# rgl-epfl/differentiable-sdf-rendering

Measured on AMD Instinct MI355X. Metric: diff-renders/sec (fwd+bwd) 256^3 SDF, 512^2, 12 views, higher is better.
Workload: dtype f32; 1 GPU; no-tex-12-hq sizes: 256^3 SDF, 12 views x 512^2, sdf_silhouette_reparam, spp primal/grad 256/64 (reference semantics, configs.py:16,19); views_total=12, views_this_rank=12, partition=whole views, spp_primal=256, spp_grad=64, schedule=primal pass and gradient sweep on two HIP streams

## Files before the change

### differentiable-sdf-rendering_amd/csrc/dsdf_items_body.h

```cpp
    static_assert(!STORE_T || !DIRECT, "STORE_T is a mode of the one-channel marches");
    constexpr int NCH = DIRECT ? 4 : 2;
    __shared__ __attribute__((aligned(16))) float wave_lds[DSDF_WAVE_LDS];
    const int lid = lane_id();
    const uint32_t npix = (uint32_t)(VB.v[0].Wb * VB.v[0].Hb);
    const uint32_t chunks = (uint32_t)__builtin_amdgcn_readfirstlane(VB.v[0].spp >> 6);
    const uint32_t n_items = (uint32_t)__builtin_amdgcn_readfirstlane((int)items[0]) * chunks;
    WaveStats wst = {0, 0, 0, 0, 0, 0, 0};
    const uint32_t sub = (blockIdx.x >> 3) & 7u, first = gridDim.x / DSDF_TICKETS;
    uint32_t share = blockIdx.x & 7u, hops = 0;
    const uint32_t my_subq = tail_subq();
    auto draw = [&](uint32_t sh) { return ticket_draw(items, sh, sub, first); };
    uint32_t item = item_of(share, blockIdx.x >> 3), next = 0;
    if (lid == 0) next = draw(share);
    while (true) {
        if (item >= n_items) {
            if (++hops == 8u) break;
            share = (share + 1u) & 7u;
            if (lid == 0) next = draw(share);
            item = (uint32_t)__builtin_amdgcn_readfirstlane((int)next);
            if (lid == 0) next = draw(share);
            continue;
        }
      {
        const uint32_t e = (uint32_t)__builtin_amdgcn_readfirstlane((int)list[item / chunks]);
        const uint32_t view = e / npix, pix = e - view * npix;
        const ViewArgs &A = VB.v[view];
        float *__restrict__ block = blocks + (size_t)view * NCH * npix;
        const int py = (int)(pix / (uint32_t)A.Wb), px = (int)(pix - (uint32_t)py * (uint32_t)A.Wb);
        const unsigned proof = skip ? (unsigned)__builtin_amdgcn_readfirstlane((int)skip[e]) : 0u;
        const bool skip_trace = (proof & (DIFF ? DSDF_PX_EMPTY_G : DSDF_PX_EMPTY)) != 0;
        const bool known_hit = !DIFF && !DIRECT && (proof & DSDF_PX_HIT) && A.integrator == DSDF_SILHOUETTE;
        const uint32_t unit = pix * chunks + item % chunks;
        const uint32_t lane = unit * 64u + (uint32_t)lid;
        auto hand_off = [&tq, my_subq, item, view, lane](auto &ho) { ho.tq = tq; ho.sub = tq.per_xcd ? my_subq : item % DSDF_TAIL_SUBQ; ho.view = view; ho.lane = lane; };
        TraceOut tr, trs, trb;
        clear_trace(tr);
        int lit = 0;
        float acc[NCH][2], win[4] = {0.f, 0.f, 0.f, 0.f};
#pragma unroll
        for (int ch = 0; ch < NCH; ++ch) { acc[ch][0] = 0.f; acc[ch][1] = 0.f; }
        const bool proven = !DIFF && !DIRECT && !STORE_T && (known_hit || skip_trace);
        Lane L;
        if (STORE_T) {
            if (!skip_trace) {
                L = lane_setup<!DIFF>(A, P, lane, px, py);
                if (DIFF) {
                    DirectFetch F;
                    if (tq.state) {
                        HandOff ho;
                        hand_off(ho);
                        trace_diff(G, P, L.ray.o, L.ray.d, L.ray.maxt, tr, F, ho);
                    } else trace_diff(G, P, L.ray.o, L.ray.d, L.ray.maxt, tr, F);
                    const Queue qv = view_queue(qall, view);
                    store_record(qv.rec + lane, qv.cap, tr);
                } else {
                    WaveCellCache F; F.taps = wave_lds; F.lid = lid;
                    if (tq.state) {
                        PlainHandOff ho;
                        hand_off(ho);
                        trace_plain(G, P, L.ray.o, L.ray.d, L.ray.maxt, tr, F, ho);
                    } else trace_plain(G, P, L.ray.o, L.ray.d, L.ray.maxt, tr, F);
                    hit_t[hit_slot(npix, A.spp, view, lane)] = tr.its_t;
                }
            }
        } else if (proven) {
            float r0, r1;
            sample_offsets(A, lane, r0, r1);
            film_accum_offsets(r0, r1, known_hit ? 1.f : 0.f, wave_lds, lid, win);
            if (known_hit) tr.its_t = 0.f;
        } else {
        L = lane_setup<!DIFF>(A, P, lane, px, py);
        if (known_hit) tr.its_t = 0.f;
        else if (!skip_trace) {
            if (DIFF) {
                DirectFetch F;
                if (!DIRECT && tq.state) {
                    HandOff ho;
                    hand_off(ho);
                    trace_diff(G, P, L.ray.o, L.ray.d, L.ray.maxt, tr, F, ho);
                } else trace_diff(G, P, L.ray.o, L.ray.d, L.ray.maxt, tr, F);
            } else {
                WaveCellCache F; F.taps = wave_lds; F.lid = lid;
                if (!DIRECT && tq.state) {
                    PlainHandOff ho;
                    hand_off(ho);
                    trace_plain(G, P, L.ray.o, L.ray.d, L.ray.maxt, tr, F, ho);
                } else trace_plain(G, P, L.ray.o, L.ray.d, L.ray.maxt, tr, F);
            }
        }
        if (DIRECT) {
            const Reproj rp = reproject(A.cam, P, L.ray.o + L.ray.d, A.W, A.H);
            float rgb[3];
            lit = direct_value(G, P, A, S, L, lane, tr.its_t, DIFF, trs, trb, rgb);
            film_accum_wave<NCH>(px, py, rp.u, rp.v, rgb, wave_lds, lid, acc);
        } else if (DIFF) {
            const Reproj rp = reproject(A.cam, P, L.ray.o + L.ray.d, A.W, A.H);
            const float val = shade_value(G, A, L, tr.its_t);
            film_accum_wave<NCH>(px, py, rp.u, rp.v, &val, wave_lds, lid, acc);
        } else {
            const float val = shade_value(G, A, L, tr.its_t);
            film_accum_offsets(L.r0, L.r1, val, wave_lds, lid, win);
        }
        }
        if (DIRECT || DIFF) { if (!STORE_T) film_flush_wave<NCH>(block, A, px, py, lid, acc); }
        else if (!STORE_T) film_flush_mfma(block, A, px, py, lid, win);
        bool need = false;
        if (DIFF && !STORE_T) {
            need = needs_backward<DIRECT>(G, P, A, L, tr, lit);
            queue_unit(view_queue(qall, view), unit, lane, need, lid, tr, DIRECT ? &trs : nullptr, (DIRECT && S.use_mis) ? &trb : nullptr);
        }
        if (STATS) add_stats(wst, tr, true, need);
        if (STATS && DIRECT) {
            wst.ssteps += wave_sum_i32(trs.steps); wst.swsteps += wave_max_i32(trs.steps); wst.srays += wave_sum_i32(trs.steps > 0 ? 1 : 0);
        }
      }
        item = (uint32_t)__builtin_amdgcn_readfirstlane((int)next);
        if (lid == 0) next = draw(share);
    }
    if (STATS) flush_stats(stats, wst, blockIdx.x, lid);
```

### differentiable-sdf-rendering_amd/csrc/dsdf_kernels.hip

```cpp
#include <hip/hip_runtime.h>
#include <stdio.h>
#include <stdlib.h>
#include <string.h>
#include <mutex>
#include <vector>
#include "dsdf_lane.h"

using namespace dsdf;

#if DSDF_XF
namespace dsdf {
__constant__ XfState g_xf_dev;
XfState g_xf_host = {{1.f, 0.f, 0.f, 0.f, 1.f, 0.f, 0.f, 0.f, 1.f}, {0.f, 0.f, 0.f}, {0.f, 0.f, 0.f}, {1.f, 1.f, 1.f}};
}
#endif

#define DSDF_BLOCK 256
#define DSDF_TSTRIDE 68
#define DSDF_TROWS 13
#define DSDF_WAVE_LDS 1104
#ifndef DSDF_PRIMAL_MINWAVES
#define DSDF_PRIMAL_MINWAVES 8
#endif

// ... 201 lines not shown
}

#define DSDF_ITEM_REGION 16384
#define DSDF_TICKETS 64
#define DSDF_ITEM_HDR (16 + 16 * DSDF_TICKETS)
__device__ __forceinline__ uint32_t ticket_draw(uint32_t *items, uint32_t sh, uint32_t sub, uint32_t first) {
    return item_of(sh, sub + 8u * (first + atomicAdd(items + 16 + 16 * (sh * 8u + sub), 1u)));
}
struct ItemOrder { int tw_log2, th_log2; uint32_t tiles_x, per_view; };

__global__ __launch_bounds__(256) void k_build_items(ViewBatch VB, int view0, int nv, const unsigned char *__restrict__ skip, unsigned far_bit,
                                                     int row0, int row1, ItemOrder O, uint32_t *__restrict__ hdr, uint32_t *__restrict__ list) {
    const ViewArgs &A = VB.v[0];
    const uint32_t npix = (uint32_t)(A.Wb * A.Hb), total = O.per_view * (uint32_t)nv;
    const uint32_t begin = blockIdx.x * DSDF_ITEM_REGION;
    const int w = threadIdx.x >> 6, lid = lane_id();
    __shared__ uint32_t wcount[4];
    __shared__ uint32_t base;
    auto entry = [&](uint32_t i) -> uint32_t {
        if (i >= total) return ~0u;
        const uint32_t gv = i / O.per_view, r = i - gv * O.per_view, view = (uint32_t)view0 + gv;
        const uint32_t tile = r >> (O.tw_log2 + O.th_log2), in = r & ((1u << (O.tw_log2 + O.th_log2)) - 1u);
        const uint32_t ty = tile / O.tiles_x, tx = tile - ty * O.tiles_x;
        const int px = (int)((tx << O.tw_log2) + (in & ((1u << O.tw_log2) - 1u))), py = (int)((ty << O.th_log2) + (in >> O.tw_log2));
        if (px >= A.Wb || py >= A.Hb || py < row0 || py >= row1) return ~0u;
        const uint32_t e = view * npix + (uint32_t)py * (uint32_t)A.Wb + (uint32_t)px;
        return (skip && (skip[e] & far_bit)) ? ~0u : e;
    };
    auto live = [&](uint32_t i) { return entry(i) != ~0u; };
    uint32_t mine = 0;
    for (uint32_t o = 0; o < DSDF_ITEM_REGION; o += 256) mine += live(begin + o + threadIdx.x) ? 1u : 0u;
    const uint32_t wsum = (uint32_t)wave_sum_i32((int)mine);
    if (lid == 0) wcount[w] = wsum;
    __syncthreads();
    if (threadIdx.x == 0) {
        const uint32_t t = wcount[0] + wcount[1] + wcount[2] + wcount[3];
        base = t ? atomicAdd(hdr, t) : 0u;
    }
    __syncthreads();
    uint32_t run = base;
    for (uint32_t o = 0; o < DSDF_ITEM_REGION; o += 256) {
        const uint32_t e = entry(begin + o + threadIdx.x);
        const bool l = e != ~0u;
        const uint64_t m = __ballot(l);
        __syncthreads();
        if (lid == 0) wcount[w] = (uint32_t)__popcll(m);
        __syncthreads();
        uint32_t before = 0, all = 0;
#pragma unroll
        for (int k = 0; k < 4; ++k) { const uint32_t c = wcount[k]; before += k < w ? c : 0u; all += c; }
        if (l) list[run + before + mask_prefix(m)] = e;
        run += all;
    }
}

#ifndef DSDF_DIRECT_PRIMAL_MINWAVES
#define DSDF_DIRECT_PRIMAL_MINWAVES 1
#endif
#ifndef DSDF_DIRECT_SWEEP_MINWAVES
#define DSDF_DIRECT_SWEEP_MINWAVES 1
#endif
template <bool DIFF, bool DIRECT, bool STATS>
__global__ __launch_bounds__(64, DIRECT ? (DIFF ? DSDF_DIRECT_SWEEP_MINWAVES : DSDF_DIRECT_PRIMAL_MINWAVES) : (DIFF ? DSDF_DIFF_MINWAVES : DSDF_PRIMAL_MINWAVES))
void k_render_items(GridView G, dsdf_params P, ViewBatch VB, float *__restrict__ blocks, Queue qall, unsigned long long *stats,
                    const unsigned char *__restrict__ skip, ShadeArgs S, TailQueue tq, uint32_t *__restrict__ items,
                    const uint32_t *__restrict__ list) {
    constexpr bool STORE_T = false;
    float *const hit_t = nullptr;
#include "dsdf_items_body.h"
}
template <bool DIFF, bool STATS>
__global__ __launch_bounds__(64, DIFF ? DSDF_DIFF_MINWAVES : DSDF_PRIMAL_MINWAVES)
void k_render_items_store(GridView G, dsdf_params P, ViewBatch VB, Queue qall, unsigned long long *stats, const unsigned char *__restrict__ skip,
                          ShadeArgs S, TailQueue tq, uint32_t *__restrict__ items, const uint32_t *__restrict__ list, float *__restrict__ hit_t) {
    constexpr bool DIRECT = false, STORE_T = true;
    float *const blocks = nullptr;
#include "dsdf_items_body.h"
}

template <int PHASE, bool DIFF>
__global__ __launch_bounds__(64) void k_direct_items(GridView G, dsdf_params P, ViewBatch VB, float *__restrict__ blocks,
                                                     const unsigned char *__restrict__ skip, ShadeArgs S, TailQueue sq, uint32_t *__restrict__ items,
                                                     const uint32_t *__restrict__ list, float *__restrict__ hit_t, Queue qall) {
    constexpr int NCH = 4;
    __shared__ __attribute__((aligned(16))) float wave_lds[DSDF_WAVE_LDS];
    const int lid = lane_id();
    const uint32_t npix = (uint32_t)(VB.v[0].Wb * VB.v[0].Hb);
    const uint32_t chunks = (uint32_t)__builtin_amdgcn_readfirstlane(VB.v[0].spp >> 6);
    const uint32_t per_item = (PHASE == 1 && !DIFF) ? chunks : 1u;
    const uint32_t n_items = (uint32_t)__builtin_amdgcn_readfirstlane((int)items[0]) * (chunks / per_item);
    const uint32_t sub = (blockIdx.x >> 3) & 7u, first = gridDim.x / DSDF_TICKETS;
    uint32_t share = blockIdx.x & 7u, hops = 0;
    const uint32_t my_subq = tail_subq();
    auto draw = [&](uint32_t sh) { return ticket_draw(items, sh, sub, first); };
    uint32_t item = item_of(share, blockIdx.x >> 3), next = 0;
    if (lid == 0) next = draw(share);
    while (true) {
        if (item >= n_items) {
            if (++hops == 8u) break;
            share = (share + 1u) & 7u;
            if (lid == 0) next = draw(share);
            item = (uint32_t)__builtin_amdgcn_readfirstlane((int)next);
            if (lid == 0) next = draw(share);
            continue;
        }
        {
// ... 937 lines not shown
    const ViewBatch &VB;
    int nv;
    GridView G;
    ShadeArgs S;
    Queue q;
    float *film;
    const unsigned char *skip;
    unsigned long long *st64;
    bool deep_skip;
    bool env_fill;
};

template <bool DIFF>
static int prefill_film(const PassCtx &c, const Batch &b) {
    int rc;
    const dim3 grid((unsigned)((c.Wb * c.Hb + 255) / 256), b.nv), blk(256);
    if (b.deep_skip && (rc = launch("k_film_ones", k_film_ones, grid, blk, c.st, b.VB, b.skip, b.film, c.row0, c.row1, b.st64))) return rc;
    if (b.env_fill && (rc = launch("k_film_env", k_film_env, grid, blk, c.st, b.VB, b.skip, b.film, c.row0, c.row1,
                                   DIFF ? DSDF_PX_EMPTY_G : DSDF_PX_EMPTY, b.S.env[0], b.S.env[1], b.S.env[2])))
        return rc;
    return DSDF_OK;
}

template <bool DIFF>
static int persistent_pass(PassCtx &c, const Workspace &ws, const Batch &b, bool wavefront) {
    int rc;
    hipStream_t st = c.st;
    const int nv = b.nv;
    const unsigned far_bit = (c.direct && !b.S.hide_emitters && !b.env_fill) ? 0u : (DIFF ? DSDF_PX_FAR_G : (DSDF_PX_FAR | (b.deep_skip ? DSDF_PX_DEEP : 0u)));
    if (hipMemsetAsync(ws.items, 0, (size_t)DSDF_MAX_GROUPS * DSDF_ITEM_HDR * sizeof(uint32_t), st) != hipSuccess)
        return fail(DSDF_ERR_LAUNCH, "hipMemsetAsync(work list) failed");
    ItemOrder O;
    {
        unsigned tile_px = DSDF_ITEM_SEG / (unsigned)(c.spp / 64);
        if (tile_px < 1) tile_px = 1;
        int lg = 0;
        while ((2u << lg) <= tile_px) ++lg;
        O.tw_log2 = (lg + 1) / 2; O.th_log2 = lg / 2;
        O.tiles_x = (unsigned)((c.Wb + (1u << O.tw_log2) - 1) >> O.tw_log2);
        const unsigned tiles_y = (unsigned)((c.Hb + (1u << O.th_log2) - 1) >> O.th_log2);
        O.per_view = (O.tiles_x * tiles_y) << (O.tw_log2 + O.th_log2);
    }
    if (DIFF && hipMemsetAsync(ws.count, 0, (size_t)nv * ws.nunits * sizeof(uint32_t), st) != hipSuccess)
        return fail(DSDF_ERR_LAUNCH, "hipMemsetAsync(queue counts) failed");
    const bool handoff = ws.tail != nullptr && (!c.direct || wavefront);
    const size_t cnt_bytes = align_up((size_t)DSDF_MAX_GROUPS * DSDF_TAIL_SUBQ * DSDF_TAIL_CNT_STRIDE * sizeof(uint32_t), 256);
    if (handoff && hipMemsetAsync(ws.tail, 0, cnt_bytes, st) != hipSuccess)
        return fail(DSDF_ERR_LAUNCH, "hipMemsetAsync(tail queue) failed");
    uint32_t *hdr = ws.items;
    uint32_t *list = ws.items + (size_t)DSDF_MAX_GROUPS * DSDF_ITEM_HDR;
    if ((rc = launch("k_build_items", k_build_items, dim3((unsigned)(((size_t)nv * O.per_view + DSDF_ITEM_REGION - 1) / DSDF_ITEM_REGION)), dim3(256), st,
                     b.VB, 0, nv, b.skip, far_bit, c.row0, c.row1, O, hdr, list)))
        return rc;
    TailQueue tq;
    memset(&tq, 0, sizeof(tq));
    if (handoff) {
        tq.cap_sub = ws.tail_cap_sub * (uint32_t)((nv + ws.group_views - 1) / ws.group_views);
        tq.per_xcd = 1u;
        tq.count = (uint32_t *)ws.tail;
        tq.state = (float *)(ws.tail + cnt_bytes);
    }
    const GridView &G = b.G;
    const ShadeArgs &S = b.S;
    const Queue &q = b.q;
    unsigned long long *st64 = b.st64;
    const dim3 grid(worker_blocks()), blk(64);
    timing_mark(0, st);
    if (wavefront)
        rc = launch("k_render_items", st64 ? k_render_items_store<DIFF, true> : k_render_items_store<DIFF, false>, grid, blk, st,
                    G, c.pp, b.VB, q, st64, b.skip, S, tq, hdr, list, ws.hit_t);
    else
        rc = launch("k_render_items", c.direct ? (st64 ? k_render_items<DIFF, true, true> : k_render_items<DIFF, true, false>)
                                               : (st64 ? k_render_items<DIFF, false, true> : k_render_items<DIFF, false, false>),
                    grid, blk, st, G, c.pp, b.VB, b.film, q, st64, b.skip, S, tq, hdr, list);
    if (rc) return rc;
    timing_mark(1, st);
    if (!handoff) return DSDF_OK;
    bool coef_beside = false;
    hipEvent_t coef_fork = nullptr;
    hipStream_t hs[2] = {st, st};
    if (DIFF && c.coef_beside && ws.count0 && helper_streams(st, hs)) {
        if (hipMemcpyAsync(ws.count0, ws.count, (size_t)nv * ws.nunits * sizeof(uint32_t), hipMemcpyDeviceToDevice, st) != hipSuccess)
            return fail(DSDF_ERR_LAUNCH, "hipMemcpyAsync(queue lengths) failed");
        coef_beside = true;
        coef_fork = next_event();
        if (!coef_fork || hipEventRecord(coef_fork, st) != hipSuccess) return fail(DSDF_ERR_LAUNCH, "coefficient stream fork failed");
    }
    const dim3 tgrid(DSDF_TAIL_SUBQ * DSDF_TAIL_BLOCKS_PER_SUBQ), tblk(256);
    unsigned long long *tst = wavefront ? nullptr : (st64 ? st64 : g_tail_stats);
    if (DIFF) rc = launch("k_tail_trace", wavefront ? k_tail_trace_diff<true> : k_tail_trace_diff<false>, tgrid, tblk, st, G, c.pp, b.VB, b.film, tq, q, tst);
    else rc = launch("k_tail_trace", k_tail_trace_plain, tgrid, tblk, st, G, c.pp, b.VB, b.film, tq, tst, wavefront ? ws.hit_t : nullptr);
    if (rc) return rc;
    if (coef_beside) {
        hipStream_t cs = hs[1];
        if (hipStreamWaitEvent(cs, coef_fork, 0) != hipSuccess) return fail(DSDF_ERR_LAUNCH, "coefficient stream fork failed");
        const dim3 cgrid((ws.nunits + DSDF_BWD_UNITS - 1) / DSDF_BWD_UNITS, nv);
        if ((rc = launch("k_backward_coef", k_backward_coef, cgrid, dim3(64), cs, G, c.pp, b.VB, q, nullptr, nullptr, ws.count0))) return rc;
        hipEvent_t join = next_event();
        if (!join || hipEventRecord(join, cs) != hipSuccess) return fail(DSDF_ERR_LAUNCH, "coefficient stream join failed");
        c.coef_done_early = true;
        if (hipStreamWaitEvent(st, join, 0) != hipSuccess) return fail(DSDF_ERR_LAUNCH, "tail stream join failed");
    }
    return DSDF_OK;
}

template <bool DIFF>
// ... 359 lines not shown
```

### differentiable-sdf-rendering_amd/csrc/dsdf_math.h

```cpp
#pragma once
#include <math.h>
#include <stdint.h>
#include "../../include/dsdf.h"

#if defined(__HIPCC__)
#define DSDF_HD __host__ __device__ __forceinline__
#else
#define DSDF_HD inline
#endif

#ifndef DSDF_FAST_RCP
#define DSDF_FAST_RCP 1
#endif

namespace dsdf {

struct V3 { float x, y, z; };
DSDF_HD V3 mk(float x, float y, float z) { V3 r; r.x = x; r.y = y; r.z = z; return r; }
DSDF_HD V3 operator+(V3 a, V3 b) { return mk(a.x + b.x, a.y + b.y, a.z + b.z); }
DSDF_HD V3 operator-(V3 a, V3 b) { return mk(a.x - b.x, a.y - b.y, a.z - b.z); }
DSDF_HD V3 operator-(V3 a) { return mk(-a.x, -a.y, -a.z); }
DSDF_HD V3 operator*(V3 a, float s) { return mk(a.x * s, a.y * s, a.z * s); }
DSDF_HD V3 operator*(float s, V3 a) { return mk(a.x * s, a.y * s, a.z * s); }
DSDF_HD V3 operator*(V3 a, V3 b) { return mk(a.x * b.x, a.y * b.y, a.z * b.z); }
// ... 579 lines not shown
            float w = eval_trace_weight(P, d, i, lo, hi, x, v, g, H, w_d);
            float inv_den = rcpf_s<1>(fminf(P.extra_thresh, sd));
            float diff = prev_sd - sd;
            ews += (diff >= 0.f) ? diff * inv_den : 0.f;
            ews = fminf(ews, 1.f);
            float cur = hit ? 0.f : sd;
            float seg = 0.5f * (cur + prev_sd);
            float winc = seg * w * ews;
            wsum += winc;
            warp_t += winc * t;
            w_d = fma3(dot(d, w_d), t_d, t * w_d);
            V3 gc = fma3(dot(d, g), t_d, t * g);
            V3 seg_d = 0.5f * (gc + prev_gc);
            V3 sd_d = drsign(v) * gc;
            V3 ewd = (prev_gc - sd_d) * inv_den;
            if (v < P.extra_thresh) ewd = ewd - (diff * inv_den * inv_den) * sd_d;
            if (diff > 0.f) ews_d = ews_d + ewd;
            if (ews >= 1.f || ews <= 0.f) ews_d = mk(0.f, 0.f, 0.f);
            w_d = w * ews_d + ews * w_d;
            w *= ews;
            V3 winc_d = w * seg_d + seg * w_d;
            mixed = mixed + t * winc_d + (w * seg) * t_d;
            t_d = t_d + gc;
            wdsum = wdsum + winc_d;
            ++i;
            t += cur;
            prev_sd = sd;
            prev_gc = gc;
            active = (t <= maxt) && !hit;
        }
    }
    C.leftover(active, t, warp_t, prev_sd, wsum, ews, t_d, prev_gc, mixed, wdsum, ews_d, i);
    out.steps = i;
    out.weight_sum = wsum;
    out.its_t = refine_hit(G, P, o, d, its_t, trace_eps, out.refine_steps, F);
    float inv = 1.f / wsum;
    warp_t *= inv;
    V3 warp_t_d = (mixed - warp_t * wdsum) * inv;
    float ww = fminf(fmaxf(wsum, 0.f), 1.f);
    V3 ww_d = (wsum > 0.f && wsum < 1.f) ? wdsum : mk(0.f, 0.f, 0.f);
    bool invalid = (wsum < 1e-7f) || !hit_box || active;
    if (invalid) {
        warp_t = INFINITY; warp_t_d = mk(0.f, 0.f, 0.f); ww = 0.f; ww_d = mk(0.f, 0.f, 0.f);
    }
    out.warp_t = warp_t; out.warp_t_d = warp_t_d; out.warp_weight = ww; out.warp_weight_d = ww_d;
}

template <class Fetch>
DSDF_HD void trace_diff(const GridView &G, const dsdf_params &P, V3 o, V3 d_in, float ray_maxt, TraceOut &out, Fetch &F) {
    MarchToEnd C;
    trace_diff(G, P, o, d_in, ray_maxt, out, F, C);
}

struct DiffMarch {
    V3 o, d;
    float t, maxt, trace_eps, its_t;
    float warp_t, prev_sd, wsum, ews;
    V3 t_d, prev_gc, mixed, wdsum, ews_d;
    int i;
    bool active, hit_box;
};

DSDF_HD DiffMarch diff_march_begin(const dsdf_params &P, V3 o, V3 d_in, float ray_maxt) {
    DiffMarch m;
    float invn = rsqf_s<2>(dot(d_in, d_in));
    m.o = o;
    m.d = d_in * invn;
    const BoxBound lo = box_lo(P), hi = box_hi(P);
    BoxHit b = bbox_ray_intersect(lo, hi, o, m.d);
    m.hit_box = b.hit && (b.mint > 0.f || b.inside);
    m.active = m.hit_box;
    m.maxt = fminf(b.maxt, ray_maxt);
    m.trace_eps = P.trace_eps * fmaxf(m.maxt, 1.f);
    m.its_t = INFINITY;
    m.t = b.inside ? 0.f : b.mint + 1e-5f;
    m.warp_t = 0.f; m.prev_sd = 0.f; m.wsum = 0.f; m.ews = 0.f;
    m.prev_gc = mk(0.f, 0.f, 0.f); m.mixed = mk(0.f, 0.f, 0.f); m.wdsum = mk(0.f, 0.f, 0.f); m.ews_d = mk(0.f, 0.f, 0.f);
    m.i = 0;
    V3 pb = fma3(m.t, m.d, o);
    V3 n = closest_axis(box_face_distance(lo, hi, pb));
    float ddn = dot(m.d, n);
    m.t_d = mk(0.f, 0.f, 0.f);
    if (!b.inside && fabsf(ddn) > 0.f) m.t_d = n * (-m.t / ddn);
    return m;
}

DSDF_HD void diff_march_step(const dsdf_params &P, DiffMarch &m, V3 x, float v, V3 g, const float H[6]) {
    const BoxBound lo = box_lo(P), hi = box_hi(P);
    const V3 d = m.d;
    const float t = m.t;
    bool hit = v < m.trace_eps;
    if (hit) m.its_t = t;
    float sd = fabsf(v);
    V3 w_d;
    float w = eval_trace_weight(P, d, m.i, lo, hi, x, v, g, H, w_d);
    float inv_den = rcpf_s<1>(fminf(P.extra_thresh, sd));
    float diff = m.prev_sd - sd;
    m.ews += (diff >= 0.f) ? diff * inv_den : 0.f;
    m.ews = fminf(m.ews, 1.f);
    float cur = hit ? 0.f : sd;
    float seg = 0.5f * (cur + m.prev_sd);
    float winc = seg * w * m.ews;
    m.wsum += winc;
    m.warp_t += winc * t;
    w_d = fma3(dot(d, w_d), m.t_d, t * w_d);
    V3 gc = fma3(dot(d, g), m.t_d, t * g);
// ... 425 lines not shown
```

### differentiable-sdf-rendering_amd/python/dsdf/_lib.py

```python
import ctypes as C
import os

_HERE = os.path.dirname(os.path.abspath(__file__))
LIB_PATH = os.environ.get('DSDF_LIB_PATH') or os.path.normpath(os.path.join(_HERE, '..', '..', 'lib', 'libdsdf.so'))

DSDF_SILHOUETTE = 0
DSDF_SIMPLE_SHADING = 1
DSDF_DIRECT = 2
DSDF_REPARAM = 1
DSDF_NO_SKIP = 2
DSDF_NO_HIT_PROOF = 4


class DsdfCamera(C.Structure):
    _fields_ = [('origin', C.c_float * 3), ('left', C.c_float * 3), ('up', C.c_float * 3),
                ('dir', C.c_float * 3), ('tan_half_fov', C.c_float), ('pad', C.c_float * 3)]


class DsdfParams(C.Structure):
    _fields_ = [('trace_eps', C.c_float), ('extra_thresh', C.c_float), ('sil_weight_offset', C.c_float),
                ('sil_weight_epsilon', C.c_float), ('bbox_delta', C.c_float), ('edge_eps', C.c_float),
                ('clamping_thresh', C.c_float), ('near_clip', C.c_float), ('far_clip', C.c_float),
                ('sdf_p', C.c_float * 3), ('weight_strategy', C.c_int), ('refine_steps', C.c_int),
                ('light_dir', C.c_float * 3), ('normalize_warp_field', C.c_int), ('max_reparam_depth', C.c_int)]


class DsdfShading(C.Structure):
    _fields_ = [('albedo', C.c_void_p), ('ax', C.c_int), ('ay', C.c_int), ('az', C.c_int),
                ('env_radiance', C.c_float * 3), ('hide_emitters', C.c_int), ('emitter_samples', C.c_void_p),
                ('grad_albedo', C.c_void_p), ('use_mis', C.c_int), ('variant', C.c_int), ('bsdf_samples', C.c_void_p),
                ('bsdf', C.c_int), ('roughness', C.c_void_p), ('rax', C.c_int), ('ray', C.c_int), ('raz', C.c_int),
                ('grad_roughness', C.c_void_p), ('bsdf_lobe_samples', C.c_void_p)]


class DsdfError(RuntimeError):
    pass


_lib = None
ABI_VERSION = 308

SYMBOLS = {
    'dsdf_version': (C.c_int, []),
    'dsdf_share_pixel_skip': (C.c_int, [C.c_void_p, C.c_size_t]),
    'dsdf_kernel_timing_arm': (C.c_int, []),
    'dsdf_tail_stats_arm': (C.c_int, [C.c_void_p]),
    'dsdf_kernel_timing_read': (C.c_int, [C.POINTER(C.c_float)]),
    'dsdf_last_error': (C.c_char_p, []),
    'dsdf_default_params': (None, [C.POINTER(DsdfParams)]),
    'dsdf_padded_size': (C.c_size_t, [C.c_int, C.c_int, C.c_int]),
    'dsdf_pad_grid': (C.c_int, [C.c_void_p, C.c_int, C.c_int, C.c_int, C.c_void_p, C.c_void_p]),
    'dsdf_eval_cubic': (C.c_int, [C.c_void_p, C.c_int, C.c_int, C.c_int, C.POINTER(DsdfParams), C.c_void_p,
                                  C.c_int64, C.c_int, C.c_void_p, C.c_void_p, C.c_void_p, C.c_void_p]),
    'dsdf_trace': (C.c_int, [C.c_void_p, C.c_int, C.c_int, C.c_int, C.POINTER(DsdfParams), C.c_void_p, C.c_void_p,
                             C.c_void_p, C.c_int64, C.c_int, C.c_void_p, C.c_void_p, C.c_void_p, C.c_void_p,
                             C.c_void_p, C.c_void_p, C.c_void_p]),
    'dsdf_warp_eval': (C.c_int, [C.c_void_p, C.c_int, C.c_int, C.c_int, C.POINTER(DsdfParams), C.c_void_p, C.c_void_p, C.c_int64,
                                 C.c_void_p, C.c_void_p, C.c_void_p, C.c_void_p, C.c_void_p, C.c_void_p, C.c_void_p, C.c_void_p,
                                 C.c_void_p, C.c_void_p]),
    'dsdf_surface_interaction': (C.c_int, [C.c_void_p, C.c_int, C.c_int, C.c_int, C.POINTER(DsdfParams), C.c_void_p, C.c_void_p,
                                           C.c_void_p, C.c_int64, C.c_void_p, C.c_void_p, C.c_void_p, C.c_void_p, C.c_void_p]),
    'dsdf_render_workspace_size': (C.c_size_t, [C.c_int, C.c_int, C.c_int, C.c_int, C.c_int]),
    'dsdf_forward_workspace_size': (C.c_size_t, [C.c_int, C.c_int, C.c_int, C.c_int, C.c_int]),
    'dsdf_cell_table_size': (C.c_size_t, [C.c_int, C.c_int, C.c_int]),
# ... 92 lines not shown
```

### differentiable-sdf-rendering_amd/python/dsdf/renderer.py

```python
import contextlib
import ctypes as C

import os

import torch

from . import _lib
from ._lib import (DSDF_DIRECT, DSDF_NO_HIT_PROOF, DSDF_NO_SKIP, DSDF_REPARAM, DSDF_SILHOUETTE, DSDF_SIMPLE_SHADING, DsdfCamera,
                   DsdfShading)

INTEGRATORS = {'sdf_silhouette_reparam': DSDF_SILHOUETTE, 'sdf_simple_shading_reparam': DSDF_SIMPLE_SHADING,
               'sdf_direct_reparam': DSDF_DIRECT,
               DSDF_SILHOUETTE: DSDF_SILHOUETTE, DSDF_SIMPLE_SHADING: DSDF_SIMPLE_SHADING, DSDF_DIRECT: DSDF_DIRECT}

STAT_NAMES = ('lanes', 'bbox_lanes', 'steps', 'hits', 'refine_steps', 'warp_active', 'queue_len', 'wave_steps',
              'tail_steps', 'tail_wave_steps', 'tail_rays')
STAT_SLOTS = 16

_workspaces = {}


def _proof_flags(empty_space_skip):
    if empty_space_skip == 'empty-only':
        return DSDF_NO_HIT_PROOF
    return 0 if empty_space_skip else DSDF_NO_SKIP

MAX_VIEWS_PER_LAUNCH = 16


def _stream():
    return C.c_void_p(torch.cuda.current_stream().cuda_stream)


def _ptr(t):
    return C.c_void_p(t.data_ptr()) if t is not None else C.c_void_p(0)


def _floats(a):
    return (C.c_float * len(a))(*[float(v) for v in a])


def _as_list(sensors):
    return list(sensors) if isinstance(sensors, (list, tuple)) else [sensors]


def _require_dev(t, name, dtype=torch.float32):
    if not isinstance(t, torch.Tensor) or not t.is_cuda:
        raise _lib.DsdfError(f"{name} must be a torch tensor on the HIP device (got {type(t).__name__}"
                             f"{'' if not isinstance(t, torch.Tensor) else ' on ' + str(t.device)}); no CPU path exists")
    if t.dtype != dtype:
        raise _lib.DsdfError(f"{name} must be {dtype}, got {t.dtype}")
    return t.contiguous()


def _workspace(device, nbytes, min_bytes=None):
    ws = _workspaces.get(device)
    if ws is not None and ws.numel() >= nbytes:
        return ws
    _workspaces.pop(device, None)
    del ws
    want = int(nbytes)
    while True:
        try:
            ws = torch.empty(want, dtype=torch.uint8, device=device)
            break
        except torch.OutOfMemoryError:
            if min_bytes is None or want <= int(min_bytes):
                raise
            torch.cuda.empty_cache()
            want = max(int(min_bytes), want // 2)
    _workspaces[device] = ws
    return ws


def release_workspaces():
    _workspaces.clear()
    _sweep_workspaces.clear()

# ... 209 lines not shown
    lib = grid.lib()
    rays_o = _require_dev(rays_o, 'rays_o'); rays_d = _require_dev(rays_d, 'rays_d'); t = _require_dev(t, 't')
    n = rays_o.shape[0]
    dev = rays_o.device
    f = lambda *s: torch.empty(*s, dtype=torch.float32, device=dev)
    out = dict(p=f(n, 3), n=f(n, 3), grad=f(n, 3), t_coef=f(n))
    with torch.cuda.device(dev):
        _lib.check(lib.dsdf_surface_interaction(_ptr(grid.padded), grid.rx, grid.ry, grid.rz, C.byref(grid.params), _ptr(rays_o),
                                                _ptr(rays_d), _ptr(t), n, _ptr(out['p']), _ptr(out['n']), _ptr(out['grad']),
                                                _ptr(out['t_coef']), _stream()))
    return out


def _views(sensors):
    sensors = _as_list(sensors)
    W, H = sensors[0].film_size()
    for s in sensors:
        if s.film_size() != (W, H):
            raise _lib.DsdfError("all sensors of one call must share the film size")
    cams = (DsdfCamera * len(sensors))(*[s.to_struct() for s in sensors])
    return sensors, cams, W, H


def _sampler_args(n_views, seeds, offsets, n_lanes):
    cseeds = None
    if seeds is not None:
        seeds = [seeds] * n_views if isinstance(seeds, int) else list(seeds)
        if len(seeds) != n_views:
            raise _lib.DsdfError("one seed per view is required")
        cseeds = (C.c_uint32 * n_views)(*[int(s) & 0xffffffff for s in seeds])
    if offsets is not None:
        offsets = _require_dev(offsets, 'offsets')
        if offsets.numel() != n_views * n_lanes * 2:
            raise _lib.DsdfError(f"offsets must hold n_views*(W+4)*(H+4)*spp*2 = {n_views * n_lanes * 2} floats, "
                                 f"got {offsets.numel()}")
        return offsets, cseeds
    if cseeds is None:
        raise _lib.DsdfError("either seeds or offsets is required")
    return None, cseeds


class _Call:

    def __init__(self, grid, sensors, spp, seeds=None, offsets=None, integrator=DSDF_SILHOUETTE, reparam=True, empty_space_skip=True,
                 shading=None, emitter_samples=None, bsdf_samples=None, grad_albedo=None):
        self.grid, self.params = grid, grid.params
        self.extended = _needs_extended(shading)
        self.lib = grid.lib(self.extended)
        self.sensors, self.cams, self.W, self.H = _views(sensors)
        self.nv, self.spp = len(self.sensors), int(spp)
        self.n_lanes = (self.W + 4) * (self.H + 4) * self.spp
        self.offsets, self.cseeds = _sampler_args(self.nv, seeds, offsets, self.n_lanes)
        self.integrator = INTEGRATORS[integrator]
        self.flags = (DSDF_REPARAM if reparam else 0) | _proof_flags(empty_space_skip)
        self.sh = self._keep = None
        if self.integrator == DSDF_DIRECT:
            if shading is None:
                raise _lib.DsdfError("sdf_direct_reparam needs shading=dsdf.Shading(albedo, ...)")
            st, keep = shading.to_struct(self.nv, self.n_lanes, emitter_samples, grad_albedo, bsdf_samples)
            self.sh, self._keep = C.byref(st), (st, keep)

    def args(self):
        g = self.grid
        return (_ptr(g.padded), g.rx, g.ry, g.rz, C.byref(self.params), self.cams, self.nv, self.W, self.H, self.spp,
                _ptr(self.offsets), self.cseeds, self.integrator, self.flags, self.sh)

    def workspace(self, diff):
        size = self.lib.dsdf_render_workspace_size if diff else self.lib.dsdf_forward_workspace_size
        extra = 0
        if not diff and self.integrator == DSDF_DIRECT:
            extra = int(self.lib.dsdf_cell_table_size(self.grid.rx, self.grid.ry, self.grid.rz)) + 256
        return _workspace(self.grid.device, size(self.W, self.H, self.spp, min(self.nv, MAX_VIEWS_PER_LAUNCH), self.integrator) + extra,
                          size(self.W, self.H, self.spp, 1, self.integrator))

    def image(self, wanted=True):
        return torch.empty(self.nv, self.H, self.W, 3, dtype=torch.float32, device=self.grid.device) if wanted else None

    def run(self, entry, *tail):
        with torch.cuda.device(self.grid.device):
            _lib.check(getattr(self.lib, entry)(*self.args(), *tail, _stream()))


def sampler_offsets(sensors, spp, seeds, mirror=False, device=None):
    lib = _lib.load()
    sensors, _, W, H = _views(sensors)
    nv = len(sensors)
    n_lanes = (W + 4) * (H + 4) * int(spp)
    _, cseeds = _sampler_args(nv, seeds, None, n_lanes)
    dev = torch.device('cuda', torch.cuda.current_device()) if device is None else torch.device(device)
    out = torch.empty(nv, n_lanes, 2, dtype=torch.float32, device=dev)
    with torch.cuda.device(dev):
        _lib.check(lib.dsdf_sampler_2d(cseeds, nv, W, H, int(spp), int(bool(mirror)), _ptr(out), _stream()))
    return out


def render_forward(grid, sensors, spp, seeds=None, offsets=None, integrator=DSDF_SILHOUETTE, reparam=True, stats=None,
                   empty_space_skip=True, shading=None, emitter_samples=None, bsdf_samples=None):
    c = _Call(grid, sensors, spp, seeds, offsets, integrator, reparam, empty_space_skip, shading, emitter_samples, bsdf_samples)
    img = c.image()
    ws = c.workspace(False)
    c.run('dsdf_render_forward', _ptr(img), _ptr(ws), ws.numel(), _ptr(stats))
    return img


AOV_NAMES = ['sdf_value', 'warp_t', 'vx', 'vy', 'div', 'i', 'weight_sum', 'weight', 'warp_t_dx', 'warp_t_dy', 'warp_t_dz']


# ... 291 lines not shown
            _lib.check(lib.dsdf_redistance_status(_ptr(ws), rx, ry, rz, _ptr(status), _stream()))
            return out.reshape(shape), status
    return out.reshape(shape)


def mesh_raycast(triangles, rays_o, rays_d, t_min=0.0):
    lib = _lib.load()
    tri = _require_dev(triangles.reshape(-1, 9), 'triangles')
    rays_o = _require_dev(rays_o, 'rays_o'); rays_d = _require_dev(rays_d, 'rays_d')
    n = rays_o.shape[0]
    t = torch.empty(n, dtype=torch.float32, device=rays_o.device)
    back = torch.empty(n, dtype=torch.int32, device=rays_o.device)
    with torch.cuda.device(rays_o.device):
        _lib.check(lib.dsdf_mesh_raycast(_ptr(tri), int(tri.shape[0]), _ptr(rays_o), _ptr(rays_d), n, C.c_float(t_min), _ptr(t), _ptr(back),
                                         _stream()))
    return t, back


def kernel_timing_arm():
    _lib.check(_lib.load().dsdf_kernel_timing_arm())


def kernel_timing_read():
    ms = C.c_float(0.0)
    _lib.check(_lib.load().dsdf_kernel_timing_read(C.byref(ms)))
    return float(ms.value)


def tail_stats_arm(stats):
    global _tail_stats_held
    if stats is not None and (stats.dtype != torch.int64 or stats.numel() < 64 * STAT_SLOTS or not stats.is_contiguous()):
        raise ValueError("tail_stats_arm: a contiguous int64 tensor of 64 x STAT_SLOTS counters (new_stats()) is expected")
    for lib in {id(l): l for l in (_lib.load(), *_lib._variants.values())}.values():
        _lib.check(lib.dsdf_tail_stats_arm(_ptr(stats) if stats is not None else None))
    _tail_stats_held = stats


_tail_stats_held = None


def new_stats(device):
    return torch.zeros(64, STAT_SLOTS, dtype=torch.int64, device=device)


def stats_dict(stats):
    tot = [int(x) for x in stats.sum(0).cpu()]
    d = dict(zip(STAT_NAMES, tot))
    d['all_steps'] = d['steps'] + d['tail_steps']
    rows = [[int(x) for x in stats[r].cpu()] for r in range(4)]
    r0, r1 = rows[0], rows[1]
    d['tail_waves'] = {'max_wave_steps': r0[11], 'max_us': r0[12] / 100.0, 'sum_us': r0[13] / 100.0, 'sum_clocks': r0[14],
                       'sum_refill_clocks': r0[15], 'refills': r1[11], 'clocks_completing': r1[12], 'clocks_claiming': r1[13],
                       'clocks_setting_up': r1[14], 'idle_lanes_at_refill': r1[15]}
    M = (1 << 64) - 1
    for name, r in (('primal_tail', rows[2]), ('sweep_tail', rows[3])):
        if r[12]:
            t0 = M - (r[11] & M)
            d['tail_waves'][name] = {'latest_start_us': (r[12] - t0) / 100.0, 'earliest_end_us': ((M - (r[13] & M)) - t0) / 100.0,
                                     'latest_end_us': (r[14] - t0) / 100.0, 'first_start_tick': t0}
    return d


def eager_sweep_enabled():
    return os.environ.get('DSDF_EAGER_SWEEP', '1') != '0'


class _RenderOp(torch.autograd.Function):

    @staticmethod
    def forward(ctx, data, grid, sensors, spp, seed, spp_grad, seed_grad, integrator, reparam, p=None, albedo=None,
                shading=None, roughness=None):
        if albedo is not None:
            shading = shading.with_albedo(albedo)
        ctx.data_shape = data.shape
        ctx.p_meta = None if p is None else (p.shape, p.dtype, p.device)
        if not grid.in_sync_with(data):
            grid.update(data)
        if p is not None:
            grid.set_translation(p)
        n = len(sensors)
        sh = shading
        want_r = sh is not None and sh.roughness is not None and roughness is not None and ctx.needs_input_grad[12]
        want_a = sh is not None and (ctx.needs_input_grad[10] or want_r)
        ctx.ga = torch.zeros_like(sh.albedo.detach(), dtype=torch.float32).contiguous() if want_a else None
        ctx.gr = None
        if want_r:
            ctx.gr = sh.grad_roughness = torch.zeros_like(sh.roughness.detach(), dtype=torch.float32).contiguous()
        ctx.gp = torch.zeros(3, dtype=torch.float32, device=grid.device) if (p is not None and ctx.needs_input_grad[9]) else None
        ctx.grid = grid
        ctx.version = grid.version
        ctx.n_backward = 0
        if not eager_sweep_enabled():
            ctx.step = None
            ctx.lazy = (list(sensors), int(spp_grad), [seed_grad + i for i in range(n)], integrator, reparam, sh, grid.version)
            return render_forward(grid, sensors, spp, seeds=[seed + i for i in range(n)], integrator=integrator, reparam=reparam, shading=sh)
        img, ctx.step = step_begin(grid, sensors, spp, spp_grad, [seed + i for i in range(n)], [seed_grad + i for i in range(n)],
                                   integrator, reparam, sh, ctx.ga)
        return img

    @staticmethod
    def backward(ctx, grad_out):
        if ctx.version != ctx.grid.version:
            raise _lib.DsdfError("the grid was updated between this render and its backward: back-propagate before the optimiser step")
        if ctx.n_backward > 0:
            for t in (ctx.gp, ctx.ga, ctx.gr):
                if t is not None:
# ... 34 lines not shown
```

### include/dsdf.h

```cpp
#ifndef DSDF_H
#define DSDF_H

#include <stddef.h>
#include <stdint.h>

#ifdef __cplusplus
extern "C" {
#endif

#define DSDF_VERSION 308
#define DSDF_STAT_SLOTS 16

enum dsdf_status {
    DSDF_OK = 0,
    DSDF_ERR_INVALID_ARG = -1,
    DSDF_ERR_WORKSPACE = -2,
    DSDF_ERR_LAUNCH = -3,
    DSDF_ERR_NO_DEVICE = -4
};

enum dsdf_integrator {
    DSDF_SILHOUETTE = 0,
    DSDF_SIMPLE_SHADING = 1,
    DSDF_DIRECT = 2
};

enum dsdf_flags {
    DSDF_REPARAM = 1,
    DSDF_NO_SKIP = 2,
    DSDF_NO_HIT_PROOF = 4
};

typedef struct dsdf_camera {
    float origin[3];
    float left[3];
    float up[3];
    float dir[3];
    float tan_half_fov;
    float pad[3];
} dsdf_camera;

typedef struct dsdf_params {
    float trace_eps;
    float extra_thresh;
    float sil_weight_offset;
    float sil_weight_epsilon;
    float bbox_delta;
    float edge_eps;
    float clamping_thresh;
    float near_clip;
    float far_clip;
    float sdf_p[3];
    int   weight_strategy;
    int   refine_steps;
    float light_dir[3];
    int   normalize_warp_field;
    int   max_reparam_depth;
} dsdf_params;

typedef struct dsdf_shading {
    const float *albedo;
    int   ax, ay, az;
    float env_radiance[3];
    int   hide_emitters;
    const float *emitter_samples;
    float *grad_albedo;
    int   use_mis;
    int   variant;
    const float *bsdf_samples;
    int   bsdf;
    const float *roughness;
    int   rax, ray, raz;
    float *grad_roughness;
    const float *bsdf_lobe_samples;
} dsdf_shading;

int         dsdf_version(void);
const char *dsdf_last_error(void);
void        dsdf_default_params(dsdf_params *p);

size_t dsdf_padded_size(int rx, int ry, int rz);

int dsdf_pad_grid(const float *data, int rx, int ry, int rz, float *padded, void *stream);
// ... 101 lines not shown
```

Before: 29.41 renders/s.

## Probe gradient-sweep pixels with a capped lite march to skip full diff traces

Adds a probe kernel that, after item lists are built, traces one representative ray per pixel with a cheap capped sphere march (no derivative tracking) and marks items whose rays finish and need no backward work. In the gradient sweep, marked items first run the lite march per lane. If the whole wave finishes and needs no backward pass, the full differentiable trace and queueing are skipped; otherwise the wave falls back to the full trace. This aims to cut expensive trace_diff work on pixels far from silhouettes. The cost is an extra probe launch, redundant lite marches for chunks that fall back, and reliance on one probe ray being representative of all of a pixel's samples.

```diff
diff --git a/differentiable-sdf-rendering_amd/csrc/dsdf_items_body.h b/differentiable-sdf-rendering_amd/csrc/dsdf_items_body.h
--- a/differentiable-sdf-rendering_amd/csrc/dsdf_items_body.h
+++ b/differentiable-sdf-rendering_amd/csrc/dsdf_items_body.h
@@ -1,5 +1,7 @@
     static_assert(!STORE_T || !DIRECT, "STORE_T is a mode of the one-channel marches");
     constexpr int NCH = DIRECT ? 4 : 2;
+    constexpr bool LITE = DIFF && !DIRECT && !STORE_T;
+    int lite_wsteps = 0, lite_fallbacks = 0;
     __shared__ __attribute__((aligned(16))) float wave_lds[DSDF_WAVE_LDS];
     const int lid = lane_id();
     const uint32_t npix = (uint32_t)(VB.v[0].Wb * VB.v[0].Hb);
@@ -22,7 +24,8 @@
             continue;
         }
       {
-        const uint32_t e = (uint32_t)__builtin_amdgcn_readfirstlane((int)list[item / chunks]);
+        const uint32_t e_raw = (uint32_t)__builtin_amdgcn_readfirstlane((int)list[item / chunks]);
+        const uint32_t e = LITE ? e_raw & ~DSDF_ITEM_LITE : e_raw;
         const uint32_t view = e / npix, pix = e - view * npix;
         const ViewArgs &A = VB.v[view];
         float *__restrict__ block = blocks + (size_t)view * NCH * npix;
@@ -41,6 +44,7 @@
         for (int ch = 0; ch < NCH; ++ch) { acc[ch][0] = 0.f; acc[ch][1] = 0.f; }
         const bool proven = !DIFF && !DIRECT && !STORE_T && (known_hit || skip_trace);
         Lane L;
+        bool lite_done = false;
         if (STORE_T) {
             if (!skip_trace) {
                 L = lane_setup<!DIFF>(A, P, lane, px, py);
@@ -70,8 +74,23 @@
             if (known_hit) tr.its_t = 0.f;
         } else {
         L = lane_setup<!DIFF>(A, P, lane, px, py);
+        if (LITE && (e_raw & DSDF_ITEM_LITE) && !skip_trace) {
+#if DSDF_LITE_CACHE
+            WaveCellCache F; F.taps = wave_lds; F.lid = lid;
+#else
+            DirectFetch F;
+#endif
+            MarchCapped cap = {(A.flags & DSDF_REPARAM) ? DSDF_LITE_CAP : 0x7fffffff};
+            const bool fin = trace_lite(G, P, L.ray.o, L.ray.d, L.ray.maxt, tr, F, cap);
+            lite_done = __ballot(!fin || needs_backward<false>(G, P, A, L, tr, 0)) == 0;
+            if (STATS) {
+                const int it = wave_max_i32(tr.steps) + wave_max_i32(tr.refine_steps);
+                lite_wsteps += it;
+                if (!lite_done) { wst.steps += wave_sum_i32(tr.steps); wst.wsteps += it; ++lite_fallbacks; }
+            }
+        }
         if (known_hit) tr.its_t = 0.f;
-        else if (!skip_trace) {
+        else if (!skip_trace && !lite_done) {
             if (DIFF) {
                 DirectFetch F;
                 if (!DIRECT && tq.state) {
@@ -106,7 +125,7 @@
         else if (!STORE_T) film_flush_mfma(block, A, px, py, lid, win);
         bool need = false;
         if (DIFF && !STORE_T) {
-            need = needs_backward<DIRECT>(G, P, A, L, tr, lit);
+            need = !lite_done && needs_backward<DIRECT>(G, P, A, L, tr, lit);
             queue_unit(view_queue(qall, view), unit, lane, need, lid, tr, DIRECT ? &trs : nullptr, (DIRECT && S.use_mis) ? &trb : nullptr);
         }
         if (STATS) add_stats(wst, tr, true, need);
@@ -118,3 +137,7 @@
         if (lid == 0) next = draw(share);
     }
     if (STATS) flush_stats(stats, wst, blockIdx.x, lid);
+    if (STATS && LITE && lid == 0 && lite_wsteps) {
+        atomicAdd(stats + DSDF_STAT_LITE_ROW * DSDF_STAT_SLOTS + 11, (unsigned long long)lite_wsteps);
+        atomicAdd(stats + DSDF_STAT_LITE_ROW * DSDF_STAT_SLOTS + 12, (unsigned long long)lite_fallbacks);
+    }
diff --git a/differentiable-sdf-rendering_amd/csrc/dsdf_kernels.hip b/differentiable-sdf-rendering_amd/csrc/dsdf_kernels.hip
--- a/differentiable-sdf-rendering_amd/csrc/dsdf_kernels.hip
+++ b/differentiable-sdf-rendering_amd/csrc/dsdf_kernels.hip
@@ -277,6 +277,31 @@
         if (l) list[run + before + mask_prefix(m)] = e;
         run += all;
     }
+}
+
+#define DSDF_ITEM_LITE 0x80000000u
+#ifndef DSDF_LITE_CACHE
+#define DSDF_LITE_CACHE 1
+#endif
+__global__ __launch_bounds__(256) void k_warp_probe(GridView G, dsdf_params P, ViewBatch VB, const unsigned char *__restrict__ skip,
+                                                    const uint32_t *__restrict__ hdr, uint32_t *__restrict__ list, int mark_all) {
+    const uint32_t i = blockIdx.x * 256u + threadIdx.x;
+    if (i >= hdr[0]) return;
+    const uint32_t e = list[i];
+    bool mark = mark_all != 0;
+    if (!mark && !(skip && (skip[e] & DSDF_PX_EMPTY_G))) {
+        const uint32_t npix = (uint32_t)(VB.v[0].Wb * VB.v[0].Hb);
+        const uint32_t view = e / npix, pix = e - view * npix;
+        const ViewArgs &A = VB.v[view];
+        const int py = (int)(pix / (uint32_t)A.Wb), px = (int)(pix - (uint32_t)py * (uint32_t)A.Wb);
+        const Lane L = lane_setup(A, P, pix * (uint32_t)A.spp, px, py);
+        DirectFetch F;
+        MarchCapped cap = {DSDF_LITE_CAP};
+        TraceOut tr;
+        const bool fin = trace_lite(G, P, L.ray.o, L.ray.d, L.ray.maxt, tr, F, cap);
+        mark = fin && !needs_backward<false>(G, P, A, L, tr, 0);
+    }
+    if (mark) list[i] = e | DSDF_ITEM_LITE;
 }
 
 #ifndef DSDF_DIRECT_PRIMAL_MINWAVES
@@ -1320,6 +1345,11 @@
     if ((rc = launch("k_build_items", k_build_items, dim3((unsigned)(((size_t)nv * O.per_view + DSDF_ITEM_REGION - 1) / DSDF_ITEM_REGION)), dim3(256), st,
                      b.VB, 0, nv, b.skip, far_bit, c.row0, c.row1, O, hdr, list)))
         return rc;
+    const int lite = (DIFF && !c.direct && !wavefront && (size_t)nv * c.Wb * c.Hb < 0x80000000ull && !(c.flags & DSDF_SWEEP_LITE_OFF))
+                         ? ((c.flags & DSDF_SWEEP_LITE_ALL) ? 2 : 1) : 0;
+    if (lite > 0 && (rc = launch("k_warp_probe", k_warp_probe, dim3((unsigned)(((size_t)nv * c.Wb * c.Hb + 255) / 256)), dim3(256), st,
+                                 b.G, c.pp, b.VB, b.skip, hdr, list, (int)(lite >= 2))))
+        return rc;
     TailQueue tq;
     memset(&tq, 0, sizeof(tq));
     if (handoff) {
diff --git a/differentiable-sdf-rendering_amd/csrc/dsdf_math.h b/differentiable-sdf-rendering_amd/csrc/dsdf_math.h
--- a/differentiable-sdf-rendering_amd/csrc/dsdf_math.h
+++ b/differentiable-sdf-rendering_amd/csrc/dsdf_math.h
@@ -655,6 +655,85 @@
     trace_diff(G, P, o, d_in, ray_maxt, out, F, C);
 }
 
+template <class B>
+DSDF_HD float eval_trace_weight_lite(const dsdf_params &P, V3 d, int i, B lo, B hi, V3 x, float v, V3 g) {
+    float n_dot_d = dot(g, d);
+    float n_dot_n = dot(g, g);
+    float ratio = n_dot_d * rcpf_s<0>(n_dot_n);
+    float denom = P.sil_weight_epsilon + fabsf(v) + P.sil_weight_offset * n_dot_d * ratio;
+    float inv_denom = rcpf_s<0>(denom);
+    float dist_w = inv_denom * inv_denom * inv_denom;
+    V3 bd_d;
+    float bd = bbox_distance_inside_d(x, lo, hi, bd_d);
+    const float bbox_eps = 0.01f;
+    float bw = i > 0 ? fminf(bd, bbox_eps) * (1.f / bbox_eps) : 1.f;
+    return dist_w * bw;
+}
+
+struct MarchCapped {
+    int left;
+    template <class Fetch> DSDF_HD bool more(const Fetch &F, bool active) { return F.any(active) && left-- > 0; }
+};
+#ifndef DSDF_LITE_CAP
+#define DSDF_LITE_CAP 64
+#endif
+
+template <class Fetch, class Ctl>
+DSDF_HD bool trace_lite(const GridView &G, const dsdf_params &P, V3 o, V3 d_in, float ray_maxt, TraceOut &out, Fetch &F, Ctl &C) {
+    float invn = rsqf_s<2>(dot(d_in, d_in));
+    V3 d = d_in * invn;
+    const BoxBound lo = box_lo(P), hi = box_hi(P);
+    BoxHit b = bbox_ray_intersect(lo, hi, o, d);
+    bool hit_box = b.hit && (b.mint > 0.f || b.inside);
+    bool active = hit_box;
+    float maxt = fminf(b.maxt, ray_maxt);
+    float trace_eps = P.trace_eps * fmaxf(maxt, 1.f);
+    float its_t = INFINITY;
+    float t = b.inside ? 0.f : b.mint + 1e-5f;
+    float warp_t = 0.f, prev_sd = 0.f, wsum = 0.f, ews = 0.f;
+    int i = 0;
+    while (C.more(F, active)) {
+        V3 x = fma3(t, d, o);
+        float v = 0.f; V3 g = mk(0.f, 0.f, 0.f); float H[6];
+        F.template eval<1>(G, x, active, v, g, H);
+        if (active) {
+            bool hit = v < trace_eps;
+            if (hit) its_t = t;
+            float sd = fabsf(v);
+            float w = eval_trace_weight_lite(P, d, i, lo, hi, x, v, g);
+            float inv_den = rcpf_s<1>(fminf(P.extra_thresh, sd));
+            float diff = prev_sd - sd;
+            ews += (diff >= 0.f) ? diff * inv_den : 0.f;
+            ews = fminf(ews, 1.f);
+            float cur = hit ? 0.f : sd;
+            float seg = 0.5f * (cur + prev_sd);
+            float winc = seg * w * ews;
+            wsum += winc;
+            warp_t += winc * t;
+            ++i;
+            t += cur;
+            prev_sd = sd;
+            active = (t <= maxt) && !hit;
+        }
+    }
+    out.steps = i;
+    out.weight_sum = wsum;
+    out.its_t = refine_hit(G, P, o, d, its_t, trace_eps, out.refine_steps, F);
+    float inv = 1.f / wsum;
+    warp_t *= inv;
+    float ww = fminf(fmaxf(wsum, 0.f), 1.f);
+    bool invalid = (wsum < 1e-7f) || !hit_box || active;
+    if (invalid) { warp_t = INFINITY; ww = 0.f; }
+    out.warp_t = warp_t; out.warp_weight = ww;
+    out.warp_t_d = mk(0.f, 0.f, 0.f); out.warp_weight_d = mk(0.f, 0.f, 0.f);
+    return !active;
+}
+template <class Fetch>
+DSDF_HD bool trace_lite(const GridView &G, const dsdf_params &P, V3 o, V3 d_in, float ray_maxt, TraceOut &out, Fetch &F) {
+    MarchToEnd C;
+    return trace_lite(G, P, o, d_in, ray_maxt, out, F, C);
+}
+
 struct DiffMarch {
     V3 o, d;
     float t, maxt, trace_eps, its_t;
diff --git a/differentiable-sdf-rendering_amd/python/dsdf/_lib.py b/differentiable-sdf-rendering_amd/python/dsdf/_lib.py
--- a/differentiable-sdf-rendering_amd/python/dsdf/_lib.py
+++ b/differentiable-sdf-rendering_amd/python/dsdf/_lib.py
@@ -10,6 +10,8 @@
 DSDF_REPARAM = 1
 DSDF_NO_SKIP = 2
 DSDF_NO_HIT_PROOF = 4
+DSDF_SWEEP_LITE_OFF = 8
+DSDF_SWEEP_LITE_ALL = 16
 
 
 class DsdfCamera(C.Structure):
diff --git a/differentiable-sdf-rendering_amd/python/dsdf/renderer.py b/differentiable-sdf-rendering_amd/python/dsdf/renderer.py
--- a/differentiable-sdf-rendering_amd/python/dsdf/renderer.py
+++ b/differentiable-sdf-rendering_amd/python/dsdf/renderer.py
@@ -6,7 +6,7 @@
 import torch
 
 from . import _lib
-from ._lib import (DSDF_DIRECT, DSDF_NO_HIT_PROOF, DSDF_NO_SKIP, DSDF_REPARAM, DSDF_SILHOUETTE, DSDF_SIMPLE_SHADING, DsdfCamera,
+from ._lib import (DSDF_DIRECT, DSDF_NO_HIT_PROOF, DSDF_NO_SKIP, DSDF_REPARAM, DSDF_SWEEP_LITE_ALL, DSDF_SWEEP_LITE_OFF, DSDF_SILHOUETTE, DSDF_SIMPLE_SHADING, DsdfCamera,
                    DsdfShading)
 
 INTEGRATORS = {'sdf_silhouette_reparam': DSDF_SILHOUETTE, 'sdf_simple_shading_reparam': DSDF_SIMPLE_SHADING,
@@ -16,6 +16,7 @@
 STAT_NAMES = ('lanes', 'bbox_lanes', 'steps', 'hits', 'refine_steps', 'warp_active', 'queue_len', 'wave_steps',
               'tail_steps', 'tail_wave_steps', 'tail_rays')
 STAT_SLOTS = 16
+STAT_LITE_ROW = 4
 
 _workspaces = {}
 
@@ -24,6 +25,11 @@
     if empty_space_skip == 'empty-only':
         return DSDF_NO_HIT_PROOF
     return 0 if empty_space_skip else DSDF_NO_SKIP
+
+def _sweep_lite_flags():
+    v = os.environ.get('DSDF_SWEEP_LITE', '1')
+    return DSDF_SWEEP_LITE_OFF if v == '0' else (DSDF_SWEEP_LITE_ALL if v == '2' else 0)
+
 
 MAX_VIEWS_PER_LAUNCH = 16
 
@@ -339,7 +345,7 @@
         self.n_lanes = (self.W + 4) * (self.H + 4) * self.spp
         self.offsets, self.cseeds = _sampler_args(self.nv, seeds, offsets, self.n_lanes)
         self.integrator = INTEGRATORS[integrator]
-        self.flags = (DSDF_REPARAM if reparam else 0) | _proof_flags(empty_space_skip)
+        self.flags = (DSDF_REPARAM if reparam else 0) | _proof_flags(empty_space_skip) | _sweep_lite_flags()
         self.sh = self._keep = None
         if self.integrator == DSDF_DIRECT:
             if shading is None:
@@ -737,6 +743,8 @@
     d['tail_waves'] = {'max_wave_steps': r0[11], 'max_us': r0[12] / 100.0, 'sum_us': r0[13] / 100.0, 'sum_clocks': r0[14],
                        'sum_refill_clocks': r0[15], 'refills': r1[11], 'clocks_completing': r1[12], 'clocks_claiming': r1[13],
                        'clocks_setting_up': r1[14], 'idle_lanes_at_refill': r1[15]}
+    lite = [int(x) for x in stats[STAT_LITE_ROW].cpu()]
+    d['sweep_lite'] = {'wave_steps': lite[11], 'fallback_chunks': lite[12]}
     M = (1 << 64) - 1
     for name, r in (('primal_tail', rows[2]), ('sweep_tail', rows[3])):
         if r[12]:
diff --git a/include/dsdf.h b/include/dsdf.h
--- a/include/dsdf.h
+++ b/include/dsdf.h
@@ -10,6 +10,7 @@
 
 #define DSDF_VERSION 308
 #define DSDF_STAT_SLOTS 16
+#define DSDF_STAT_LITE_ROW 4
 
 enum dsdf_status {
     DSDF_OK = 0,
@@ -28,7 +29,9 @@
 enum dsdf_flags {
     DSDF_REPARAM = 1,
     DSDF_NO_SKIP = 2,
-    DSDF_NO_HIT_PROOF = 4
+    DSDF_NO_HIT_PROOF = 4,
+    DSDF_SWEEP_LITE_OFF = 8,
+    DSDF_SWEEP_LITE_ALL = 16
 };
 
 typedef struct dsdf_camera {
```

Result: no change. 29.61 renders/s (median of 6 runs) (+0.7%).
